# thelaycon/lazzaro

Measured on AMD Instinct MI355X. Metric: search_memories QPS + recall@10 on 10M x d=768 index; consolidate turns/sec, higher is better.
Workload: dtype bf16 encoder; int8 scan -> bf16 re-score -> fp32 re-rank; 1 GPU; global_batch=1024, seq_len=32, parallelism=tenant-dp1

## Files before the change

### csrc/kernels/search.hip

```cpp
#include "lzk_tile.h"

#include <cstdlib>

namespace {

constexpr int BM = 128;
constexpr int BN = 128;
constexpr int BK = 64;
constexpr int NT = 256;
constexpr int TILE_ELEMS = BM * BK;

__device__ __forceinline__ int swz_off(int row, int kc) {
  return row * BK + ((kc ^ ((row >> 1) & 7)) << 3);
}

template <int K>
struct TopK {
  float s[K];
  int i[K];
  __device__ __forceinline__ void init() {
#pragma unroll
    for (int j = 0; j < K; ++j) { s[j] = LZK_NEG_INF; i[j] = -1; }
  }
  __device__ __forceinline__ void push(float v, int r) {
    if (v > s[K - 1]) {
#pragma unroll
      for (int j = K - 1; j > 0; --j) {
        bool up = v > s[j - 1];
        bool here = v > s[j];
        float ns = up ? s[j - 1] : (here ? v : s[j]);
        int ni = up ? i[j - 1] : (here ? r : i[j]);
        s[j] = ns; i[j] = ni;
      }
      if (v > s[0]) { s[0] = v; i[0] = r; }
    }
  }
};

template <int K, bool HAS_BIAS, bool HAS_LABEL, bool GLDS>
__global__ __launch_bounds__(NT, 2) void flat_topk_kernel(
    const u16* __restrict__ X, long ldx, int nrows,
    const u16* __restrict__ Qm, long ldq, int nq,
    const float* __restrict__ bias, const int* __restrict__ row_label,
    const int* __restrict__ q_label, float alpha, int D,
    int rows_per_chunk, int n_chunks, int n_qblocks,
    float* __restrict__ out_s, int* __restrict__ out_i, const int* __restrict__ q_active) {
  extern __shared__ __attribute__((aligned(16))) u16 smem[];
  const int tid = threadIdx.x;
  const int lane = tid & 63;
  const int wave = tid >> 6;
  const int wrow = wave >> 1, wcol = wave & 1;
  const int h = lane >> 5, l32 = lane & 31;

  const int logical = xcd_remap(blockIdx.x, gridDim.x);
  const int chunk = logical / n_qblocks;
  const int qb = logical % n_qblocks;
  if (chunk >= n_chunks) return;
  const int q0 = qb * BN;
  if (q_active) {
    int any = 0;
    for (int t = tid; t < BN; t += NT) any |= (q0 + t < nq) && q_active[q0 + t];
    if (!__syncthreads_or(any)) return;
  }
  const int row_lo = chunk * rows_per_chunk;
  const int row_hi = min(nrows, row_lo + rows_per_chunk);
  const int ntiles = (row_hi > row_lo) ? (row_hi - row_lo + BM - 1) / BM : 0;
  const int KSTEPS = D / BK;
  const int T = ntiles * KSTEPS;

  int qlab[2] = {-1, -1};
  if (HAS_LABEL) {
#pragma unroll
    for (int cb = 0; cb < 2; ++cb) {
      int q = q0 + wcol * 64 + cb * 32 + l32;
      qlab[cb] = (q < nq) ? q_label[q] : -1;
    }
  }

  TopK<K> top[2];
  top[0].init(); top[1].init();

  const int srow = tid >> 3;
  const int skc = tid & 7;
  const u16* xsrc[4];
  const u16* qsrc[4];
  int soff[4];
#pragma unroll
  for (int i = 0; i < 4; ++i) {
    int r = srow + 32 * i;
    int q = min(q0 + r, nq - 1);
    qsrc[i] = Qm + (long)q * ldq + skc * 8;
    soff[i] = swz_off(r, skc);
  }
  auto set_xsrc = [&](int rt) {
#pragma unroll
    for (int i = 0; i < 4; ++i) {
      int r = row_lo + rt * BM + srow + 32 * i;
      r = min(r, nrows - 1);
      xsrc[i] = X + (long)r * ldx + skc * 8;
    }
  };

  const int wave_u = __builtin_amdgcn_readfirstlane(wave);
  const u16* gx[4];
  const u16* gq[4];
  int gpiece[4];
#pragma unroll
  for (int i = 0; i < 4; ++i) {
    const int c = wave_u * 4 + i;
    const int row = 8 * c + (lane >> 3);
    const int kc = (lane & 7) ^ ((row >> 1) & 7);
    gq[i] = Qm + (long)min(q0 + row, nq - 1) * ldq + kc * 8;
    gx[i] = X;
    gpiece[i] = c * 512;
  }
  auto set_gx = [&](int rt_) {
#pragma unroll
    for (int i = 0; i < 4; ++i) {
      const int row = 8 * (wave_u * 4 + i) + (lane >> 3);
      const int kc = (lane & 7) ^ ((row >> 1) & 7);
      gx[i] = X + (long)min(row_lo + rt_ * BM + row, nrows - 1) * ldx + kc * 8;
    }
  };
  float* ebias_g = reinterpret_cast<float*>(smem + 4 * TILE_ELEMS);
  int* elab_g = reinterpret_cast<int*>(ebias_g + 2 * BM);
  auto gissue = [&](int buf, int ks_, int rt_) {
    u16* xs = smem + buf * 2 * TILE_ELEMS;
    u16* qs = xs + TILE_ELEMS;
#pragma unroll
    for (int i = 0; i < 4; ++i) {
      __builtin_amdgcn_global_load_lds((lzk::gbl_void_t*)(gx[i] + ks_ * BK), (lzk::lds_void_t*)(xs + gpiece[i]), 16, 0, 0);
      __builtin_amdgcn_global_load_lds((lzk::gbl_void_t*)(gq[i] + ks_ * BK), (lzk::lds_void_t*)(qs + gpiece[i]), 16, 0, 0);
    }
    if ((HAS_BIAS || HAS_LABEL) && ks_ == 0 && wave_u == 0) {
#pragma unroll
      for (int h2 = 0; h2 < 2; ++h2) {
        const int r = min(row_lo + rt_ * BM + h2 * 64 + lane, nrows - 1);
        if (HAS_BIAS)
          __builtin_amdgcn_global_load_lds((lzk::gbl_void_t*)(bias + r), (lzk::lds_void_t*)(ebias_g + (rt_ & 1) * BM + h2 * 64), 4, 0, 0);
        if (HAS_LABEL)
          __builtin_amdgcn_global_load_lds((lzk::gbl_void_t*)(row_label + r), (lzk::lds_void_t*)(elab_g + (rt_ & 1) * BM + h2 * 64), 4, 0, 0);
      }
    }
  };

  u16x8 rx[4], rq[4];
  float rbias = 0.f;
  int rlab = 0;
  float* ebias = reinterpret_cast<float*>(smem + 4 * TILE_ELEMS);
  int* elab = reinterpret_cast<int*>(ebias + 2 * BM);
  auto gload = [&](int ks, int rt_) {
#pragma unroll
    for (int i = 0; i < 4; ++i) {
      rx[i] = *reinterpret_cast<const u16x8*>(xsrc[i] + ks * BK);
      rq[i] = *reinterpret_cast<const u16x8*>(qsrc[i] + ks * BK);
    }
    if ((HAS_BIAS || HAS_LABEL) && ks == 0 && tid < BM) {
      int r = min(row_lo + rt_ * BM + tid, nrows - 1);
      if (HAS_BIAS) rbias = bias[r];
      if (HAS_LABEL) rlab = row_label[r];
    }
  };
  auto swrite = [&](int buf, int ks, int rt_) {
    u16* xs = smem + buf * 2 * TILE_ELEMS;
    u16* qs = xs + TILE_ELEMS;
#pragma unroll
    for (int i = 0; i < 4; ++i) {
      *reinterpret_cast<u16x8*>(xs + soff[i]) = rx[i];
      *reinterpret_cast<u16x8*>(qs + soff[i]) = rq[i];
    }
    if ((HAS_BIAS || HAS_LABEL) && ks == 0 && tid < BM) {
      if (HAS_BIAS) ebias[(rt_ & 1) * BM + tid] = rbias;
      if (HAS_LABEL) elab[(rt_ & 1) * BM + tid] = rlab;
    }
  };

  f32x16 acc[2][2];

  if (T > 0) {
    if (GLDS) {
      set_gx(0);
      gissue(0, 0, 0);
      lzk::vm_drain();
    } else {
      set_xsrc(0);
      gload(0, 0);
      swrite(0, 0, 0);
    }
  }
  __syncthreads();

  int rt = 0, ks = 0;
  for (int t = 0; t < T; ++t) {
    const bool has_next = (t + 1 < T);
    const int nks = (ks + 1 == KSTEPS) ? 0 : ks + 1;
    const int nrt = (ks + 1 == KSTEPS) ? rt + 1 : rt;
    if (has_next) {
      if (GLDS) {
        if (nks == 0) set_gx(nrt);
        gissue((t + 1) & 1, nks, nrt);
      } else {
        if (nks == 0) set_xsrc(nrt);
        gload(nks, nrt);
      }
    }
    if (ks == 0) {
#pragma unroll
      for (int a = 0; a < 2; ++a)
#pragma unroll
        for (int b = 0; b < 2; ++b)
#pragma unroll
          for (int e = 0; e < 16; ++e) acc[a][b][e] = 0.f;
    }
    if (GLDS) __builtin_amdgcn_s_setprio(1);
    {
      const u16* xs = smem + (t & 1) * 2 * TILE_ELEMS;
      const u16* qs = xs + TILE_ELEMS;
#pragma unroll
      for (int s = 0; s < BK / 16; ++s) {
        bf16x8 af[2], bfr[2];
#pragma unroll
        for (int rb = 0; rb < 2; ++rb) {
          int r = wrow * 64 + rb * 32 + l32;
          af[rb] = *reinterpret_cast<const bf16x8*>(xs + swz_off(r, 2 * s + h));
        }
#pragma unroll
        for (int cb = 0; cb < 2; ++cb) {
          int r = wcol * 64 + cb * 32 + l32;
          bfr[cb] = *reinterpret_cast<const bf16x8*>(qs + swz_off(r, 2 * s + h));
        }
#pragma unroll
        for (int rb = 0; rb < 2; ++rb)
#pragma unroll
          for (int cb = 0; cb < 2; ++cb)
            acc[rb][cb] = __builtin_amdgcn_mfma_f32_32x32x16_bf16(af[rb], bfr[cb], acc[rb][cb], 0, 0, 0);
      }
    }
    if (GLDS) __builtin_amdgcn_s_setprio(0);
    if (ks == KSTEPS - 1) {
      const int lrow0 = wrow * 64 + 4 * h;
      const int tile0 = row_lo + rt * BM + lrow0;
      const float* eb = ebias + (rt & 1) * BM + lrow0;
      const int* el = elab + (rt & 1) * BM + lrow0;
      const bool full_tile = row_lo + (rt + 1) * BM <= row_hi;
      auto score = [&](int rb, int cb, int e) -> float {
        float x = alpha * acc[rb][cb][e];
        if (HAS_BIAS) x += eb[rb * 32 + 8 * (e >> 2) + (e & 3)];
        bool ok = true;
        if (!full_tile) ok = tile0 + rb * 32 + (e & 3) + 8 * (e >> 2) < row_hi;
        if (HAS_LABEL) ok = ok && (qlab[cb] < 0 || el[rb * 32 + 8 * (e >> 2) + (e & 3)] == qlab[cb]);
        return ok ? x : LZK_NEG_INF;
      };
#pragma unroll
      for (int rb = 0; rb < 2; ++rb) {
#pragma unroll
        for (int cb = 0; cb < 2; ++cb) {
          float m = LZK_NEG_INF;
#pragma unroll
          for (int e = 0; e < 16; ++e) m = fmaxf(m, score(rb, cb, e));
          if (m > top[cb].s[K - 1]) {
#pragma unroll
            for (int e = 0; e < 16; ++e)
              top[cb].push(score(rb, cb, e), tile0 + rb * 32 + (e & 3) + 8 * (e >> 2));
          }
        }
      }
    }
    if (GLDS) {
      lzk::vm_drain();
    } else if (has_next) {
      swrite((t + 1) & 1, nks, nrt);
    }
    __syncthreads();
    ks = nks; rt = nrt;
  }

  float* ms = reinterpret_cast<float*>(smem);
  int* mi = reinterpret_cast<int*>(smem) + BN * 4 * K;
#pragma unroll
  for (int cb = 0; cb < 2; ++cb) {
    int ql = wcol * 64 + cb * 32 + l32;
    int li = wrow * 2 + h;
#pragma unroll
    for (int j = 0; j < K; ++j) {
      ms[(ql * 4 + li) * K + j] = top[cb].s[j];
      mi[(ql * 4 + li) * K + j] = top[cb].i[j];
    }
  }
  __syncthreads();
  if (tid < BN) {
    const int ql = tid;
    const int q = q0 + ql;
    if (q < nq) {
      int p0 = 0, p1 = 0, p2 = 0, p3 = 0;
      const float* bs = ms + ql * 4 * K;
      const int* bi = mi + ql * 4 * K;
      long obase = ((long)q * n_chunks + chunk) * K;
      for (int j = 0; j < K; ++j) {
        float bsv = LZK_NEG_INF; int biv = -1; int w = -1;
        if (p0 < K) { float s = bs[0 * K + p0]; int i = bi[0 * K + p0]; if (w < 0 || better(s, i, bsv, biv)) { bsv = s; biv = i; w = 0; } }
        if (p1 < K) { float s = bs[1 * K + p1]; int i = bi[1 * K + p1]; if (w < 0 || better(s, i, bsv, biv)) { bsv = s; biv = i; w = 1; } }
        if (p2 < K) { float s = bs[2 * K + p2]; int i = bi[2 * K + p2]; if (w < 0 || better(s, i, bsv, biv)) { bsv = s; biv = i; w = 2; } }
        if (p3 < K) { float s = bs[3 * K + p3]; int i = bi[3 * K + p3]; if (w < 0 || better(s, i, bsv, biv)) { bsv = s; biv = i; w = 3; } }
        p0 += (w == 0); p1 += (w == 1); p2 += (w == 2); p3 += (w == 3);
        out_s[obase + j] = bsv;
        out_i[obase + j] = (bsv == LZK_NEG_INF) ? -1 : biv;
      }
    }
  }
}

template <int K>
__global__ __launch_bounds__(256) void topk_merge_kernel(
    const float* __restrict__ ps, const int* __restrict__ pi, int ncand, int nq,
    int kout, long idx_offset, float* __restrict__ os, long* __restrict__ oi, const int* __restrict__ q_active) {
  const int lane = threadIdx.x & 63;
  const int q = blockIdx.x * 4 + (threadIdx.x >> 6);
  if (q >= nq) return;
  if (q_active && !q_active[q]) return;
  TopK<K> top;
  top.init();
  const float* s = ps + (long)q * ncand;
  const int* ix = pi + (long)q * ncand;
  for (int c = lane; c < ncand; c += 64) {
    float v = s[c];
    int r = ix[c];
    if (r < 0) continue;
    if (better(v, r, top.s[K - 1], top.i[K - 1] < 0 ? 0x7fffffff : top.i[K - 1])) {
#pragma unroll
      for (int j = K - 1; j > 0; --j) {
        int ij1 = top.i[j - 1] < 0 ? 0x7fffffff : top.i[j - 1];
        int ij = top.i[j] < 0 ? 0x7fffffff : top.i[j];
        bool up = better(v, r, top.s[j - 1], ij1);
        bool here = better(v, r, top.s[j], ij);
        float ns = up ? top.s[j - 1] : (here ? v : top.s[j]);
        int ni = up ? top.i[j - 1] : (here ? r : top.i[j]);
        top.s[j] = ns; top.i[j] = ni;
      }
      int i0 = top.i[0] < 0 ? 0x7fffffff : top.i[0];
      if (better(v, r, top.s[0], i0)) { top.s[0] = v; top.i[0] = r; }
    }
  }
// ... 144 lines not shown
  if (D % BK != 0 || nq <= 0 || nrows <= 0) return (int)hipErrorInvalidValue;
  hipStream_t st = (hipStream_t)stream;
  const u16* x = (const u16*)X;
  const u16* q = (const u16*)Qm;
#define LZK_KS(KK) return launch_flat<KK>(x, ldx, nrows, q, ldq, nq, bias, row_label, q_label, alpha, D, n_chunks, ps, pi, st, q_active)
  switch (kslot) {
    case 1: LZK_KS(1);
    case 2: LZK_KS(2);
    case 4: LZK_KS(4);
    case 8: LZK_KS(8);
    case 10: LZK_KS(10);
    case 16: LZK_KS(16);
    default: return (int)hipErrorInvalidValue;
  }
#undef LZK_KS
}

LZK_EXPORT int lzk_flat_topk_partial(const void* X, long ldx, int nrows, const void* Qm, long ldq,
                                     int nq, const float* bias, const int* row_label,
                                     const int* q_label, float alpha, int D, int kslot,
                                     int n_chunks, float* ps, int* pi, void* stream) {
  return flat_partial(X, ldx, nrows, Qm, ldq, nq, bias, row_label, q_label, alpha, D, kslot, n_chunks, ps, pi,
                      stream, nullptr);
}

LZK_EXPORT int lzk_flat_topk_partial_masked(const void* X, long ldx, int nrows, const void* Qm, long ldq, int nq,
                                            const float* bias, const int* row_label, const int* q_label,
                                            float alpha, int D, int kslot, int n_chunks, float* ps, int* pi,
                                            const int* q_active, void* stream) {
  return flat_partial(X, ldx, nrows, Qm, ldq, nq, bias, row_label, q_label, alpha, D, kslot, n_chunks, ps, pi,
                      stream, q_active);
}

static int topk_merge(const float* ps, const int* pi, int ncand, int nq, int kslot, int kout, long idx_offset,
                      float* os, long* oi, void* stream, const int* q_active) {
  hipStream_t st = (hipStream_t)stream;
  dim3 grid((nq + 3) / 4), block(256);
  if (kout > kslot) return (int)hipErrorInvalidValue;
#define LZK_M(KK) hipLaunchKernelGGL(topk_merge_kernel<KK>, grid, block, 0, st, ps, pi, ncand, nq, kout, idx_offset, os, oi, q_active)
  switch (kslot) {
    case 1: LZK_M(1); break;
    case 2: LZK_M(2); break;
    case 4: LZK_M(4); break;
    case 8: LZK_M(8); break;
    case 10: LZK_M(10); break;
    case 16: LZK_M(16); break;
    default: return (int)hipErrorInvalidValue;
  }
#undef LZK_M
  return (int)hipGetLastError();
}

LZK_EXPORT int lzk_topk_merge(const float* ps, const int* pi, int ncand, int nq, int kslot,
                              int kout, long idx_offset, float* os, long* oi, void* stream) {
  return topk_merge(ps, pi, ncand, nq, kslot, kout, idx_offset, os, oi, stream, nullptr);
}

LZK_EXPORT int lzk_topk_merge64(const float* ps, const long* pi, int ncand, int nq, int kout, float* os, long* oi,
                                void* stream) {
  if (nq <= 0) return 0;
  if (kout < 1 || ncand < 0) return (int)hipErrorInvalidValue;
  hipStream_t st = (hipStream_t)stream;
  dim3 grid((nq + 3) / 4), block(256);
#define LZK_M64(KK) hipLaunchKernelGGL(topk_merge64_kernel<KK>, grid, block, 0, st, ps, pi, ncand, nq, kout, os, oi)
  if (kout <= 4) LZK_M64(4);
  else if (kout <= 10) LZK_M64(10);
// ... 12 lines not shown
```

### csrc/kernels/search256.hip

```cpp
#include "lzk_g256.h"

#include <cstdlib>
#include <cfloat>
#include <map>
#include <mutex>

LZK_DEBUG_STATE(search256)

namespace {

using namespace g256;

constexpr int kStampTiles = 32;
__device__ unsigned long long* g_stamps = nullptr;

template <bool HAS_BIAS, bool HAS_LABEL>
__global__ __launch_bounds__(NT, 1) void flat_cand_kernel(
    const u16* __restrict__ X, long ldx, int nrows, const u16* __restrict__ Qm, long ldq, int nq, int D,
    const float* __restrict__ bias, const int* __restrict__ row_label, const int* __restrict__ q_label,
    float alpha, const float* __restrict__ thr, int n_qt, int cap, int* __restrict__ cnt,
    float* __restrict__ cs, int* __restrict__ ci) {
  extern __shared__ __attribute__((aligned(16))) u16 smem[];
  const int logical = xcd_remap(blockIdx.x, gridDim.x);
  const int rt = logical / n_qt, qt = logical % n_qt;
  const int r0 = rt * BM, q0 = qt * BN;

  Stager st;
  st.setup(X, ldx, r0, nrows, Qm, ldq, q0, nq);
  f32x4 acc[8][4];
  mainloop(smem, st, D / BK, acc);

  const int lane = threadIdx.x & 63;
  const int wave = __builtin_amdgcn_readfirstlane(threadIdx.x >> 6);
// ... 31 lines not shown
        s[e] = ok ? s[e] : LZK_NEG_INF;
        m = fmaxf(m, s[e]);
      }
      if (m >= th[j]) {
#pragma unroll
        for (int e = 0; e < 4; ++e) {
          if (s[e] >= th[j] && s[e] != LZK_NEG_INF) {
            const int pos = atomicAdd(cnt + qq[j], 1);
            if (pos < cap) {
              cs[(long)qq[j] * cap + pos] = s[e];
              ci[(long)qq[j] * cap + pos] = rb + e;
            }
          }
        }
      }
    }
  }
}

constexpr int EPI_OFF = 8 * HALF;
constexpr int EPI_ARRAYS = 7;
constexpr int CNT_OFF = EPI_OFF + 2 * EPI_ARRAYS * 256 * 2;
constexpr int CAND_P_LDS = LDS_BYTES + 2 * EPI_ARRAYS * 256 * 4 + 16;
typedef __attribute__((address_space(3))) int lds_int;

struct BlkCands {
  int4* buf;
  int cap;
  int* cnt;
  const float* rs = nullptr;
  const float* qs = nullptr;
};

__device__ __forceinline__ float i8_prod(int v, float rs) { return __fmul_rn((float)v, rs); }
__device__ __forceinline__ float i8_score(float al, float p, float b) { return __fmaf_rn(al, p, b); }

template <bool HAS_BIAS, bool HAS_LABEL, bool DUAL, int OPT = 0, class MMA = MmaBf16>
__global__ __launch_bounds__(NT, 1) void flat_cand_persistent_kernel(
    const u16* __restrict__ X, long ldx, int nrows, const u16* __restrict__ Qm, long ldq, int nq, int D,
    const float* __restrict__ bias, const int* __restrict__ row_label, const int* __restrict__ q_label,
    float alpha, const float* __restrict__ thr, int n_qt, int n_tiles, int cap, int* __restrict__ cnt,
    float* __restrict__ cs, int* __restrict__ ci, const float* __restrict__ thr2, int* __restrict__ cnt2,
    float* __restrict__ cs2, int* __restrict__ ci2, BlkCands blk) {
  static_assert(!DUAL || HAS_LABEL, "dual search needs labels");
  extern __shared__ __attribute__((aligned(16))) u16 smem[];
  float* epi = reinterpret_cast<float*>(smem + EPI_OFF);
  lds_int* lcnt = (lds_int*)(smem + CNT_OFF);
  if (threadIdx.x == 0) *lcnt = 0;
  const int lane = threadIdx.x & 63;
  const int wave = __builtin_amdgcn_readfirstlane(threadIdx.x >> 6);
  const int wr = wave >> 2, wc = wave & 3;
  const int KS = D / BK;

  TileWalk walk;
  walk.init(n_tiles);
  int tile = walk.next;
  if (!walk.valid(tile)) {
    if (threadIdx.x == 0) blk.cnt[blockIdx.x] = 0;
    return;
  }

  auto stage_epi = [&](int tl, int par) {
    const int r0 = (tl / n_qt) * BM, q0 = (tl % n_qt) * BN;
#pragma unroll
    for (int g = wave; g < 4 * EPI_ARRAYS; g += 8) {
      const int a = g >> 2, c = g & 3;
      const bool need = a == 0 || (a == 1 && HAS_BIAS) || ((a == 2 || a == 3) && HAS_LABEL) || (a == 4 && DUAL) ||
                        ((a == 5 || a == 6) && MMA::kInt);
// ... 1323 lines not shown
```

### lazzaro_amd/ops/search.py

```python
from __future__ import annotations

import os

import numpy as np
import torch

from . import _lib

TARGET_WGS = 512


def _ref_topk(X, Q, k, bias=None, row_label=None, q_label=None, alpha=1.0, idx_offset=0,
              chunk=1 << 16):
    nq = Q.shape[0]
    n = X.shape[0]
    dev = X.device
    best_s = torch.full((nq, 0), float("-inf"), device=dev)
    best_i = torch.zeros((nq, 0), dtype=torch.long, device=dev)
    Qf = Q.float()
    for c0 in range(0, n, chunk):
        c1 = min(n, c0 + chunk)
        s = alpha * (Qf @ X[c0:c1].float().T)
        if bias is not None:
            s = s + bias[c0:c1].float()[None, :]
# ... 102 lines not shown
        return s[:, 0], i[:, 0].to(torch.int32)
    assert X.dtype == torch.bfloat16 and Q.dtype == torch.bfloat16
    assert X.shape[1] == D and D % 64 == 0 and X.stride(1) == 1 and Q.stride(1) == 1
    dev = X.device
    if N == 0 or nq == 0:
        return torch.full((nq,), float("-inf"), device=dev), torch.full((nq,), -1, dtype=torch.int32, device=dev)
    ws = torch.empty(nq, dtype=torch.int64, device=dev)
    score = torch.empty(nq, dtype=torch.float32, device=dev)
    row = torch.empty(nq, dtype=torch.int32, device=dev)
    _lib.check(_lib.lib().lzk_flat_top1(X.data_ptr(), X.stride(0), N, Q.data_ptr(), Q.stride(0), nq, D, ws.data_ptr(),
                                        score.data_ptr(), row.data_ptr(), _lib.stream_ptr(dev)), "lzk_flat_top1")
    return score, row


def _flat_topk_lane(X, Q, k, kslot, bias, row_label, q_label, alpha, idx_offset, n_chunks):
    L = _lib.lib()
    nq, D = Q.shape
    N = X.shape[0]
    if n_chunks:
        rpc = -(-(-(-N // n_chunks)) // 128) * 128
        nch = -(-N // rpc)
    else:
        nch = L.lzk_flat_topk_chunks(N, nq, TARGET_WGS)
    dev = X.device
    part = nq * nch * kslot
    ws = _ws.get(dev, part * 8)
    ps = ws[: part * 4].view(torch.float32)
    pi = ws[part * 4: part * 8].view(torch.int32)
    st = _lib.stream_ptr(dev)
    rc = L.lzk_flat_topk_partial(X.data_ptr(), X.stride(0), N, Q.data_ptr(), Q.stride(0), nq,
                                 _lib.ptr(bias), _lib.ptr(row_label), _lib.ptr(q_label),
                                 float(alpha), D, kslot, nch, ps.data_ptr(), pi.data_ptr(), st)
    _lib.check(rc, "lzk_flat_topk_partial")
    ncand = nch * kslot
    G = _merge_groups(nq, nch)
    if G > 1:
        os1 = torch.empty((nq * G, kslot), dtype=torch.float32, device=dev)
        oi1 = torch.empty((nq * G, kslot), dtype=torch.long, device=dev)
        _lib.check(L.lzk_topk_merge(ps.data_ptr(), pi.data_ptr(), ncand // G, nq * G, kslot, kslot, 0,
                                    os1.data_ptr(), oi1.data_ptr(), st), "lzk_topk_merge")
        ps, pi, ncand = os1, oi1.to(torch.int32), G * kslot
    os_ = torch.empty((nq, k), dtype=torch.float32, device=dev)
    oi = torch.empty((nq, k), dtype=torch.long, device=dev)
    rc = L.lzk_topk_merge(ps.data_ptr(), pi.data_ptr(), ncand, nq, kslot, int(k),
                          int(idx_offset), os_.data_ptr(), oi.data_ptr(), st)
    _lib.check(rc, "lzk_topk_merge")
    return os_, oi


def _merge_groups(nq: int, nch: int) -> int:
    if nq >= 64 or nch < 16:
        return 1
    for G in range(min(64, nch // 8, 512 // max(nq, 1)), 1, -1):
        if nch % G == 0:
            return G
    return 1


def _sample_threshold(X, Q, k, kslot, bias, row_label, q_label, alpha, S):
    N = X.shape[0]
    bs = bias[:N:S].contiguous() if bias is not None else None
    ls = row_label[:N:S].contiguous() if row_label is not None else None
    ts, _ = _flat_topk_lane(X[::S], Q, kslot, kslot, bs, ls, q_label, alpha, 0, None)
    thr = ts[:, k - 1].contiguous()
    thr = thr - 2e-4 * (1.0 + thr.abs())
    return torch.nan_to_num(thr, nan=float("-inf"))
# ... 232 lines not shown


def quantize_i8_rows(x: torch.Tensor, out: torch.Tensor = None, scale_out: torch.Tensor = None):
    xf = x.float()
    amax = xf.abs().amax(1)
    s = torch.where(amax > 0, amax / 127.0, torch.zeros_like(amax))
    den = torch.where(amax > 0, s, torch.ones_like(amax))
    q = torch.round(xf / den[:, None]).clamp_(-127, 127).to(torch.int8)
    if out is not None:
        out[:, : q.shape[1]] = q
        q = out
    if scale_out is not None:
        scale_out.copy_(s)
        s = scale_out
    return q, s


def i8_query(q16: torch.Tensor, d: int, sumsq: torch.Tensor, n_sumsq: int, smax: torch.Tensor, alpha: float,
             z: float, xn: float = 1.0):
    nq, Dp = q16.shape
    dev = q16.device
    q8 = torch.empty((nq, Dp), dtype=torch.int8, device=dev)
    qs = torch.empty(nq, dtype=torch.float32, device=dev)
    margin = torch.empty(nq, dtype=torch.float32, device=dev)
    margin_rig = torch.empty(nq, dtype=torch.float32, device=dev)
    q16 = q16.contiguous()
    _lib.check(_lib.lib().lzk_i8_query(q16.data_ptr(), q16.stride(0), nq, Dp, int(d), sumsq.data_ptr(),
                                       1.0 / max(int(n_sumsq), 1), smax.data_ptr(), abs(float(alpha)), float(z),
                                       float(xn), q8.data_ptr(), q8.stride(0), qs.data_ptr(), margin.data_ptr(),
                                       margin_rig.data_ptr(), _lib.stream_ptr(dev)), "lzk_i8_query")
    return q8, qs, margin, margin_rig


def flat_topk_i8(X8: torch.Tensor, rscale: torch.Tensor, Q8: torch.Tensor, qscale: torch.Tensor,
                 X16: torch.Tensor, Q16: torch.Tensor, k: int, *, bias=None, alpha: float = 1.0, margin=None,
                 margin_rig=None):
    L = _lib.lib()
    nq, Dp = Q16.shape
    N = X16.shape[0]
    kslot = L.lzk_flat_topk_kslot(int(k))
    assert kslot > 0 and X8.dtype == torch.int8 and Q8.dtype == torch.int8 and Dp % 128 == 0 and Dp <= 1024
    assert X8.shape[1] == Dp and X8.stride(1) == 1 and Q8.stride(1) == 1 and X8.shape[0] >= N
    assert rscale.dtype == torch.float32 and qscale.dtype == torch.float32 and rscale.shape[0] >= N
    assert alpha > 0
    dev = X16.device
    if margin_rig is None:
        margin_rig = margin
    narrow = nq < NARROW_MAX_Q and SCAN8_NARROW and Dp % 64 == 0
    S = max(1, min(CAND_STRIDE_NARROW if narrow else CAND_STRIDE, N // max(16 * kslot, 1)))
    J = SPEC_J_NARROW if narrow else SPEC_J
    spec = 0 < J < k and S >= SPEC_MIN_STRIDE
    bs = bias[:N:S].contiguous() if bias is not None else None
    ts, _ = _flat_topk_lane(X16[::S], Q16, kslot, kslot, bs, None, None, alpha, 0, None)
    cap = max(NARROW_CAP if narrow else 2048, 16 * kslot * S)
    cnt, cs, ci = _cand_lists(dev, nq, cap, 0, zero=False)
    thr = torch.empty(nq, dtype=torch.float32, device=dev)
    cert = torch.empty(nq, dtype=torch.float32, device=dev)
    mg = margin.float().contiguous() if margin is not None else None
    mr = margin_rig.float().contiguous() if margin_rig is not None else None
    _lib.check(L.lzk_thr_prep(ts.data_ptr(), ts.stride(0), (J if spec else k) - 1, _lib.ptr(mg), _lib.ptr(mr), nq,
                              thr.data_ptr(), cert.data_ptr(), cnt.data_ptr(), _lib.stream_ptr(dev)), "lzk_thr_prep")
    qs = qscale.contiguous()
    need = torch.empty(nq, dtype=torch.int32, device=dev)
    chk = (cert, k, cap + 1, need)
    if narrow:
        _scan8_narrow(X8[:N], rscale[:N], Q8, qs, bias, alpha, thr, kslot, 2 * S, cap, (cnt, cs, ci))
    else:
        grid = L.lzk_cand_grid_f8(N, nq)
        bbuf, bcap, bcnt = _blk_records(dev, grid, nq, kslot, 2 * S, 1)
        st = _lib.stream_ptr(dev)
        _lib.check(L.lzk_flat_cand_i8(X8.data_ptr(), X8.stride(0), N, Q8.data_ptr(), Q8.stride(0), nq, Dp,
                                      _lib.ptr(bias), rscale.data_ptr(), qs.data_ptr(), float(alpha), thr.data_ptr(),
                                      cap, cnt.data_ptr(), cs.data_ptr(), ci.data_ptr(), bbuf.data_ptr(), bcap,
                                      bcnt.data_ptr(), st), "lzk_flat_cand_i8")
        _lib.check(L.lzk_cand_gather(bbuf.data_ptr(), bcap, bcnt.data_ptr(), grid, cap, nq, cnt.data_ptr(),
                                     cs.data_ptr(), ci.data_ptr(), None, None, None, st), "lzk_cand_gather")
    _rescore_above_cut(X16, Q16, k, kslot, bias, alpha, margin_rig, cnt, cs, ci, cap, chk=chk)
    return _select_with_fallback(X16, Q16, k, kslot, bias, None, None, alpha, 0, cnt, cs, ci, cap, need=need)


def _cert_tau(thr: torch.Tensor, margin_rig: torch.Tensor, floor: float = None,
              floor_tol: float = 0.0) -> torch.Tensor:
    t = thr + margin_rig if margin_rig is not None else thr
    fl_ok = (t <= float(floor) + float(floor_tol)) if floor is not None else None
    t = t + 1e-6 * (1.0 + t.abs())
    if fl_ok is not None:
# ... 367 lines not shown
```

Baseline: 85750 queries/s.

## Compute strided sample top-k threshold with int8 MFMA directly on X8

Adds a sample_topk_i8 kernel that scores every S-th row of the int8 index with i32 MFMA and per-row/per-query scales, then merges the partials. This replaces the bf16 sampled top-k, which first materialised a strided copy of the bias and read the bf16 rows X16[::S]. The intent is to halve the bytes read by the threshold-estimation pass and drop the strided gather and copy. In exchange the thresholds now come from quantized scores, which may differ slightly from the bf16 ones and can change how many candidates pass the filter. It is enabled by default through an environment flag.

```diff
diff --git a/csrc/include/lzk_i8score.h b/csrc/include/lzk_i8score.h
--- /dev/null
+++ b/csrc/include/lzk_i8score.h
@@ -0,0 +1,5 @@
+#pragma once
+#include "lzk_common.h"
+
+__device__ __forceinline__ float i8_prod(int v, float rs) { return __fmul_rn((float)v, rs); }
+__device__ __forceinline__ float i8_score(float al, float p, float b) { return __fmaf_rn(al, p, b); }
diff --git a/csrc/kernels/search.hip b/csrc/kernels/search.hip
--- a/csrc/kernels/search.hip
+++ b/csrc/kernels/search.hip
@@ -1,4 +1,5 @@
 #include "lzk_tile.h"
+#include "lzk_i8score.h"
 
 #include <cstdlib>
 
@@ -37,244 +38,13 @@
   }
 };
 
-template <int K, bool HAS_BIAS, bool HAS_LABEL, bool GLDS>
-__global__ __launch_bounds__(NT, 2) void flat_topk_kernel(
-    const u16* __restrict__ X, long ldx, int nrows,
-    const u16* __restrict__ Qm, long ldq, int nq,
-    const float* __restrict__ bias, const int* __restrict__ row_label,
-    const int* __restrict__ q_label, float alpha, int D,
-    int rows_per_chunk, int n_chunks, int n_qblocks,
-    float* __restrict__ out_s, int* __restrict__ out_i, const int* __restrict__ q_active) {
-  extern __shared__ __attribute__((aligned(16))) u16 smem[];
+template <int K>
+__device__ __forceinline__ void merge_lane_lists(u16* smem, const TopK<K> (&top)[2], int q0, int nq, int n_chunks,
+                                                 int chunk, float* __restrict__ out_s, int* __restrict__ out_i) {
   const int tid = threadIdx.x;
-  const int lane = tid & 63;
-  const int wave = tid >> 6;
+  const int lane = tid & 63, wave = tid >> 6;
   const int wrow = wave >> 1, wcol = wave & 1;
   const int h = lane >> 5, l32 = lane & 31;
-
-  const int logical = xcd_remap(blockIdx.x, gridDim.x);
-  const int chunk = logical / n_qblocks;
-  const int qb = logical % n_qblocks;
-  if (chunk >= n_chunks) return;
-  const int q0 = qb * BN;
-  if (q_active) {
-    int any = 0;
-    for (int t = tid; t < BN; t += NT) any |= (q0 + t < nq) && q_active[q0 + t];
-    if (!__syncthreads_or(any)) return;
-  }
-  const int row_lo = chunk * rows_per_chunk;
-  const int row_hi = min(nrows, row_lo + rows_per_chunk);
-  const int ntiles = (row_hi > row_lo) ? (row_hi - row_lo + BM - 1) / BM : 0;
-  const int KSTEPS = D / BK;
-  const int T = ntiles * KSTEPS;
-
-  int qlab[2] = {-1, -1};
-  if (HAS_LABEL) {
-#pragma unroll
-    for (int cb = 0; cb < 2; ++cb) {
-      int q = q0 + wcol * 64 + cb * 32 + l32;
-      qlab[cb] = (q < nq) ? q_label[q] : -1;
-    }
-  }
-
-  TopK<K> top[2];
-  top[0].init(); top[1].init();
-
-  const int srow = tid >> 3;
-  const int skc = tid & 7;
-  const u16* xsrc[4];
-  const u16* qsrc[4];
-  int soff[4];
-#pragma unroll
-  for (int i = 0; i < 4; ++i) {
-    int r = srow + 32 * i;
-    int q = min(q0 + r, nq - 1);
-    qsrc[i] = Qm + (long)q * ldq + skc * 8;
-    soff[i] = swz_off(r, skc);
-  }
-  auto set_xsrc = [&](int rt) {
-#pragma unroll
-    for (int i = 0; i < 4; ++i) {
-      int r = row_lo + rt * BM + srow + 32 * i;
-      r = min(r, nrows - 1);
-      xsrc[i] = X + (long)r * ldx + skc * 8;
-    }
-  };
-
-  const int wave_u = __builtin_amdgcn_readfirstlane(wave);
-  const u16* gx[4];
-  const u16* gq[4];
-  int gpiece[4];
-#pragma unroll
-  for (int i = 0; i < 4; ++i) {
-    const int c = wave_u * 4 + i;
-    const int row = 8 * c + (lane >> 3);
-    const int kc = (lane & 7) ^ ((row >> 1) & 7);
-    gq[i] = Qm + (long)min(q0 + row, nq - 1) * ldq + kc * 8;
-    gx[i] = X;
-    gpiece[i] = c * 512;
-  }
-  auto set_gx = [&](int rt_) {
-#pragma unroll
-    for (int i = 0; i < 4; ++i) {
-      const int row = 8 * (wave_u * 4 + i) + (lane >> 3);
-      const int kc = (lane & 7) ^ ((row >> 1) & 7);
-      gx[i] = X + (long)min(row_lo + rt_ * BM + row, nrows - 1) * ldx + kc * 8;
-    }
-  };
-  float* ebias_g = reinterpret_cast<float*>(smem + 4 * TILE_ELEMS);
-  int* elab_g = reinterpret_cast<int*>(ebias_g + 2 * BM);
-  auto gissue = [&](int buf, int ks_, int rt_) {
-    u16* xs = smem + buf * 2 * TILE_ELEMS;
-    u16* qs = xs + TILE_ELEMS;
-#pragma unroll
-    for (int i = 0; i < 4; ++i) {
-      __builtin_amdgcn_global_load_lds((lzk::gbl_void_t*)(gx[i] + ks_ * BK), (lzk::lds_void_t*)(xs + gpiece[i]), 16, 0, 0);
-      __builtin_amdgcn_global_load_lds((lzk::gbl_void_t*)(gq[i] + ks_ * BK), (lzk::lds_void_t*)(qs + gpiece[i]), 16, 0, 0);
-    }
-    if ((HAS_BIAS || HAS_LABEL) && ks_ == 0 && wave_u == 0) {
-#pragma unroll
-      for (int h2 = 0; h2 < 2; ++h2) {
-        const int r = min(row_lo + rt_ * BM + h2 * 64 + lane, nrows - 1);
-        if (HAS_BIAS)
-          __builtin_amdgcn_global_load_lds((lzk::gbl_void_t*)(bias + r), (lzk::lds_void_t*)(ebias_g + (rt_ & 1) * BM + h2 * 64), 4, 0, 0);
-        if (HAS_LABEL)
-          __builtin_amdgcn_global_load_lds((lzk::gbl_void_t*)(row_label + r), (lzk::lds_void_t*)(elab_g + (rt_ & 1) * BM + h2 * 64), 4, 0, 0);
-      }
-    }
-  };
-
-  u16x8 rx[4], rq[4];
-  float rbias = 0.f;
-  int rlab = 0;
-  float* ebias = reinterpret_cast<float*>(smem + 4 * TILE_ELEMS);
-  int* elab = reinterpret_cast<int*>(ebias + 2 * BM);
-  auto gload = [&](int ks, int rt_) {
-#pragma unroll
-    for (int i = 0; i < 4; ++i) {
-      rx[i] = *reinterpret_cast<const u16x8*>(xsrc[i] + ks * BK);
-      rq[i] = *reinterpret_cast<const u16x8*>(qsrc[i] + ks * BK);
-    }
-    if ((HAS_BIAS || HAS_LABEL) && ks == 0 && tid < BM) {
-      int r = min(row_lo + rt_ * BM + tid, nrows - 1);
-      if (HAS_BIAS) rbias = bias[r];
-      if (HAS_LABEL) rlab = row_label[r];
-    }
-  };
-  auto swrite = [&](int buf, int ks, int rt_) {
-    u16* xs = smem + buf * 2 * TILE_ELEMS;
-    u16* qs = xs + TILE_ELEMS;
-#pragma unroll
-    for (int i = 0; i < 4; ++i) {
-      *reinterpret_cast<u16x8*>(xs + soff[i]) = rx[i];
-      *reinterpret_cast<u16x8*>(qs + soff[i]) = rq[i];
-    }
-    if ((HAS_BIAS || HAS_LABEL) && ks == 0 && tid < BM) {
-      if (HAS_BIAS) ebias[(rt_ & 1) * BM + tid] = rbias;
-      if (HAS_LABEL) elab[(rt_ & 1) * BM + tid] = rlab;
-    }
-  };
-
-  f32x16 acc[2][2];
-
-  if (T > 0) {
-    if (GLDS) {
-      set_gx(0);
-      gissue(0, 0, 0);
-      lzk::vm_drain();
-    } else {
-      set_xsrc(0);
-      gload(0, 0);
-      swrite(0, 0, 0);
-    }
-  }
-  __syncthreads();
-
-  int rt = 0, ks = 0;
-  for (int t = 0; t < T; ++t) {
-    const bool has_next = (t + 1 < T);
-    const int nks = (ks + 1 == KSTEPS) ? 0 : ks + 1;
-    const int nrt = (ks + 1 == KSTEPS) ? rt + 1 : rt;
-    if (has_next) {
-      if (GLDS) {
-        if (nks == 0) set_gx(nrt);
-        gissue((t + 1) & 1, nks, nrt);
-      } else {
-        if (nks == 0) set_xsrc(nrt);
-        gload(nks, nrt);
-      }
-    }
-    if (ks == 0) {
-#pragma unroll
-      for (int a = 0; a < 2; ++a)
-#pragma unroll
-        for (int b = 0; b < 2; ++b)
-#pragma unroll
-          for (int e = 0; e < 16; ++e) acc[a][b][e] = 0.f;
-    }
-    if (GLDS) __builtin_amdgcn_s_setprio(1);
-    {
-      const u16* xs = smem + (t & 1) * 2 * TILE_ELEMS;
-      const u16* qs = xs + TILE_ELEMS;
-#pragma unroll
-      for (int s = 0; s < BK / 16; ++s) {
-        bf16x8 af[2], bfr[2];
-#pragma unroll
-        for (int rb = 0; rb < 2; ++rb) {
-          int r = wrow * 64 + rb * 32 + l32;
-          af[rb] = *reinterpret_cast<const bf16x8*>(xs + swz_off(r, 2 * s + h));
-        }
-#pragma unroll
-        for (int cb = 0; cb < 2; ++cb) {
-          int r = wcol * 64 + cb * 32 + l32;
-          bfr[cb] = *reinterpret_cast<const bf16x8*>(qs + swz_off(r, 2 * s + h));
-        }
-#pragma unroll
-        for (int rb = 0; rb < 2; ++rb)
-#pragma unroll
-          for (int cb = 0; cb < 2; ++cb)
-            acc[rb][cb] = __builtin_amdgcn_mfma_f32_32x32x16_bf16(af[rb], bfr[cb], acc[rb][cb], 0, 0, 0);
-      }
-    }
-    if (GLDS) __builtin_amdgcn_s_setprio(0);
-    if (ks == KSTEPS - 1) {
-      const int lrow0 = wrow * 64 + 4 * h;
-      const int tile0 = row_lo + rt * BM + lrow0;
-      const float* eb = ebias + (rt & 1) * BM + lrow0;
-      const int* el = elab + (rt & 1) * BM + lrow0;
-      const bool full_tile = row_lo + (rt + 1) * BM <= row_hi;
-      auto score = [&](int rb, int cb, int e) -> float {
-        float x = alpha * acc[rb][cb][e];
-        if (HAS_BIAS) x += eb[rb * 32 + 8 * (e >> 2) + (e & 3)];
-        bool ok = true;
-        if (!full_tile) ok = tile0 + rb * 32 + (e & 3) + 8 * (e >> 2) < row_hi;
-        if (HAS_LABEL) ok = ok && (qlab[cb] < 0 || el[rb * 32 + 8 * (e >> 2) + (e & 3)] == qlab[cb]);
-        return ok ? x : LZK_NEG_INF;
-      };
-#pragma unroll
-      for (int rb = 0; rb < 2; ++rb) {
-#pragma unroll
-        for (int cb = 0; cb < 2; ++cb) {
-          float m = LZK_NEG_INF;
-#pragma unroll
-          for (int e = 0; e < 16; ++e) m = fmaxf(m, score(rb, cb, e));
-          if (m > top[cb].s[K - 1]) {
-#pragma unroll
-            for (int e = 0; e < 16; ++e)
-              top[cb].push(score(rb, cb, e), tile0 + rb * 32 + (e & 3) + 8 * (e >> 2));
-          }
-        }
-      }
-    }
-    if (GLDS) {
-      lzk::vm_drain();
-    } else if (has_next) {
-      swrite((t + 1) & 1, nks, nrt);
-    }
-    __syncthreads();
-    ks = nks; rt = nrt;
-  }
-
   float* ms = reinterpret_cast<float*>(smem);
   int* mi = reinterpret_cast<int*>(smem) + BN * 4 * K;
 #pragma unroll
@@ -308,6 +78,409 @@
       }
     }
   }
+}
+
+template <int K, bool HAS_BIAS, bool HAS_LABEL, bool GLDS>
+__global__ __launch_bounds__(NT, 2) void flat_topk_kernel(
+    const u16* __restrict__ X, long ldx, int nrows,
+    const u16* __restrict__ Qm, long ldq, int nq,
+    const float* __restrict__ bias, const int* __restrict__ row_label,
+    const int* __restrict__ q_label, float alpha, int D,
+    int rows_per_chunk, int n_chunks, int n_qblocks,
+    float* __restrict__ out_s, int* __restrict__ out_i, const int* __restrict__ q_active) {
+  extern __shared__ __attribute__((aligned(16))) u16 smem[];
+  const int tid = threadIdx.x;
+  const int lane = tid & 63;
+  const int wave = tid >> 6;
+  const int wrow = wave >> 1, wcol = wave & 1;
+  const int h = lane >> 5, l32 = lane & 31;
+
+  const int logical = xcd_remap(blockIdx.x, gridDim.x);
+  const int chunk = logical / n_qblocks;
+  const int qb = logical % n_qblocks;
+  if (chunk >= n_chunks) return;
+  const int q0 = qb * BN;
+  if (q_active) {
+    int any = 0;
+    for (int t = tid; t < BN; t += NT) any |= (q0 + t < nq) && q_active[q0 + t];
+    if (!__syncthreads_or(any)) return;
+  }
+  const int row_lo = chunk * rows_per_chunk;
+  const int row_hi = min(nrows, row_lo + rows_per_chunk);
+  const int ntiles = (row_hi > row_lo) ? (row_hi - row_lo + BM - 1) / BM : 0;
+  const int KSTEPS = D / BK;
+  const int T = ntiles * KSTEPS;
+
+  int qlab[2] = {-1, -1};
+  if (HAS_LABEL) {
+#pragma unroll
+    for (int cb = 0; cb < 2; ++cb) {
+      int q = q0 + wcol * 64 + cb * 32 + l32;
+      qlab[cb] = (q < nq) ? q_label[q] : -1;
+    }
+  }
+
+  TopK<K> top[2];
+  top[0].init(); top[1].init();
+
+  const int srow = tid >> 3;
+  const int skc = tid & 7;
+  const u16* xsrc[4];
+  const u16* qsrc[4];
+  int soff[4];
+#pragma unroll
+  for (int i = 0; i < 4; ++i) {
+    int r = srow + 32 * i;
+    int q = min(q0 + r, nq - 1);
+    qsrc[i] = Qm + (long)q * ldq + skc * 8;
+    soff[i] = swz_off(r, skc);
+  }
+  auto set_xsrc = [&](int rt) {
+#pragma unroll
+    for (int i = 0; i < 4; ++i) {
+      int r = row_lo + rt * BM + srow + 32 * i;
+      r = min(r, nrows - 1);
+      xsrc[i] = X + (long)r * ldx + skc * 8;
+    }
+  };
+
+  const int wave_u = __builtin_amdgcn_readfirstlane(wave);
+  const u16* gx[4];
+  const u16* gq[4];
+  int gpiece[4];
+#pragma unroll
+  for (int i = 0; i < 4; ++i) {
+    const int c = wave_u * 4 + i;
+    const int row = 8 * c + (lane >> 3);
+    const int kc = (lane & 7) ^ ((row >> 1) & 7);
+    gq[i] = Qm + (long)min(q0 + row, nq - 1) * ldq + kc * 8;
+    gx[i] = X;
+    gpiece[i] = c * 512;
+  }
+  auto set_gx = [&](int rt_) {
+#pragma unroll
+    for (int i = 0; i < 4; ++i) {
+      const int row = 8 * (wave_u * 4 + i) + (lane >> 3);
+      const int kc = (lane & 7) ^ ((row >> 1) & 7);
+      gx[i] = X + (long)min(row_lo + rt_ * BM + row, nrows - 1) * ldx + kc * 8;
+    }
+  };
+  float* ebias_g = reinterpret_cast<float*>(smem + 4 * TILE_ELEMS);
+  int* elab_g = reinterpret_cast<int*>(ebias_g + 2 * BM);
+  auto gissue = [&](int buf, int ks_, int rt_) {
+    u16* xs = smem + buf * 2 * TILE_ELEMS;
+    u16* qs = xs + TILE_ELEMS;
+#pragma unroll
+    for (int i = 0; i < 4; ++i) {
+      __builtin_amdgcn_global_load_lds((lzk::gbl_void_t*)(gx[i] + ks_ * BK), (lzk::lds_void_t*)(xs + gpiece[i]), 16, 0, 0);
+      __builtin_amdgcn_global_load_lds((lzk::gbl_void_t*)(gq[i] + ks_ * BK), (lzk::lds_void_t*)(qs + gpiece[i]), 16, 0, 0);
+    }
+    if ((HAS_BIAS || HAS_LABEL) && ks_ == 0 && wave_u == 0) {
+#pragma unroll
+      for (int h2 = 0; h2 < 2; ++h2) {
+        const int r = min(row_lo + rt_ * BM + h2 * 64 + lane, nrows - 1);
+        if (HAS_BIAS)
+          __builtin_amdgcn_global_load_lds((lzk::gbl_void_t*)(bias + r), (lzk::lds_void_t*)(ebias_g + (rt_ & 1) * BM + h2 * 64), 4, 0, 0);
+        if (HAS_LABEL)
+          __builtin_amdgcn_global_load_lds((lzk::gbl_void_t*)(row_label + r), (lzk::lds_void_t*)(elab_g + (rt_ & 1) * BM + h2 * 64), 4, 0, 0);
+      }
+    }
+  };
+
+  u16x8 rx[4], rq[4];
+  float rbias = 0.f;
+  int rlab = 0;
+  float* ebias = reinterpret_cast<float*>(smem + 4 * TILE_ELEMS);
+  int* elab = reinterpret_cast<int*>(ebias + 2 * BM);
+  auto gload = [&](int ks, int rt_) {
+#pragma unroll
+    for (int i = 0; i < 4; ++i) {
+      rx[i] = *reinterpret_cast<const u16x8*>(xsrc[i] + ks * BK);
+      rq[i] = *reinterpret_cast<const u16x8*>(qsrc[i] + ks * BK);
+    }
+    if ((HAS_BIAS || HAS_LABEL) && ks == 0 && tid < BM) {
+      int r = min(row_lo + rt_ * BM + tid, nrows - 1);
+      if (HAS_BIAS) rbias = bias[r];
+      if (HAS_LABEL) rlab = row_label[r];
+    }
+  };
+  auto swrite = [&](int buf, int ks, int rt_) {
+    u16* xs = smem + buf * 2 * TILE_ELEMS;
+    u16* qs = xs + TILE_ELEMS;
+#pragma unroll
+    for (int i = 0; i < 4; ++i) {
+      *reinterpret_cast<u16x8*>(xs + soff[i]) = rx[i];
+      *reinterpret_cast<u16x8*>(qs + soff[i]) = rq[i];
+    }
+    if ((HAS_BIAS || HAS_LABEL) && ks == 0 && tid < BM) {
+      if (HAS_BIAS) ebias[(rt_ & 1) * BM + tid] = rbias;
+      if (HAS_LABEL) elab[(rt_ & 1) * BM + tid] = rlab;
+    }
+  };
+
+  f32x16 acc[2][2];
+
+  if (T > 0) {
+    if (GLDS) {
+      set_gx(0);
+      gissue(0, 0, 0);
+      lzk::vm_drain();
+    } else {
+      set_xsrc(0);
+      gload(0, 0);
+      swrite(0, 0, 0);
+    }
+  }
+  __syncthreads();
+
+  int rt = 0, ks = 0;
+  for (int t = 0; t < T; ++t) {
+    const bool has_next = (t + 1 < T);
+    const int nks = (ks + 1 == KSTEPS) ? 0 : ks + 1;
+    const int nrt = (ks + 1 == KSTEPS) ? rt + 1 : rt;
+    if (has_next) {
+      if (GLDS) {
+        if (nks == 0) set_gx(nrt);
+        gissue((t + 1) & 1, nks, nrt);
+      } else {
+        if (nks == 0) set_xsrc(nrt);
+        gload(nks, nrt);
+      }
+    }
+    if (ks == 0) {
+#pragma unroll
+      for (int a = 0; a < 2; ++a)
+#pragma unroll
+        for (int b = 0; b < 2; ++b)
+#pragma unroll
+          for (int e = 0; e < 16; ++e) acc[a][b][e] = 0.f;
+    }
+    if (GLDS) __builtin_amdgcn_s_setprio(1);
+    {
+      const u16* xs = smem + (t & 1) * 2 * TILE_ELEMS;
+      const u16* qs = xs + TILE_ELEMS;
+#pragma unroll
+      for (int s = 0; s < BK / 16; ++s) {
+        bf16x8 af[2], bfr[2];
+#pragma unroll
+        for (int rb = 0; rb < 2; ++rb) {
+          int r = wrow * 64 + rb * 32 + l32;
+          af[rb] = *reinterpret_cast<const bf16x8*>(xs + swz_off(r, 2 * s + h));
+        }
+#pragma unroll
+        for (int cb = 0; cb < 2; ++cb) {
+          int r = wcol * 64 + cb * 32 + l32;
+          bfr[cb] = *reinterpret_cast<const bf16x8*>(qs + swz_off(r, 2 * s + h));
+        }
+#pragma unroll
+        for (int rb = 0; rb < 2; ++rb)
+#pragma unroll
+          for (int cb = 0; cb < 2; ++cb)
+            acc[rb][cb] = __builtin_amdgcn_mfma_f32_32x32x16_bf16(af[rb], bfr[cb], acc[rb][cb], 0, 0, 0);
+      }
+    }
+    if (GLDS) __builtin_amdgcn_s_setprio(0);
+    if (ks == KSTEPS - 1) {
+      const int lrow0 = wrow * 64 + 4 * h;
+      const int tile0 = row_lo + rt * BM + lrow0;
+      const float* eb = ebias + (rt & 1) * BM + lrow0;
+      const int* el = elab + (rt & 1) * BM + lrow0;
+      const bool full_tile = row_lo + (rt + 1) * BM <= row_hi;
+      auto score = [&](int rb, int cb, int e) -> float {
+        float x = alpha * acc[rb][cb][e];
+        if (HAS_BIAS) x += eb[rb * 32 + 8 * (e >> 2) + (e & 3)];
+        bool ok = true;
+        if (!full_tile) ok = tile0 + rb * 32 + (e & 3) + 8 * (e >> 2) < row_hi;
+        if (HAS_LABEL) ok = ok && (qlab[cb] < 0 || el[rb * 32 + 8 * (e >> 2) + (e & 3)] == qlab[cb]);
+        return ok ? x : LZK_NEG_INF;
+      };
+#pragma unroll
+      for (int rb = 0; rb < 2; ++rb) {
+#pragma unroll
+        for (int cb = 0; cb < 2; ++cb) {
+          float m = LZK_NEG_INF;
+#pragma unroll
+          for (int e = 0; e < 16; ++e) m = fmaxf(m, score(rb, cb, e));
+          if (m > top[cb].s[K - 1]) {
+#pragma unroll
+            for (int e = 0; e < 16; ++e)
+              top[cb].push(score(rb, cb, e), tile0 + rb * 32 + (e & 3) + 8 * (e >> 2));
+          }
+        }
+      }
+    }
+    if (GLDS) {
+      lzk::vm_drain();
+    } else if (has_next) {
+      swrite((t + 1) & 1, nks, nrt);
+    }
+    __syncthreads();
+    ks = nks; rt = nrt;
+  }
+
+  merge_lane_lists<K>(smem, top, q0, nq, n_chunks, chunk, out_s, out_i);
+}
+
+template <int K, bool HAS_BIAS>
+__global__ __launch_bounds__(NT, 2) void sample_topk_i8_kernel(
+    const int8_t* __restrict__ X, long ldx, int ns, int S,
+    const int8_t* __restrict__ Qm, long ldq, int nq,
+    const float* __restrict__ rscale, const float* __restrict__ qscale, const float* __restrict__ bias,
+    float alpha, int D, int rows_per_chunk, int n_chunks, int n_qblocks,
+    float* __restrict__ out_s, int* __restrict__ out_i) {
+  typedef int i32x4 __attribute__((ext_vector_type(4)));
+  typedef int i32x16 __attribute__((ext_vector_type(16)));
+  constexpr int BKB = 2 * BK;
+  extern __shared__ __attribute__((aligned(16))) u16 smem[];
+  const int tid = threadIdx.x;
+  const int lane = tid & 63;
+  const int wave = tid >> 6;
+  const int wrow = wave >> 1, wcol = wave & 1;
+  const int h = lane >> 5, l32 = lane & 31;
+
+  const int logical = xcd_remap(blockIdx.x, gridDim.x);
+  const int chunk = logical / n_qblocks;
+  const int qb = logical % n_qblocks;
+  if (chunk >= n_chunks) return;
+  const int q0 = qb * BN;
+  const int row_lo = chunk * rows_per_chunk;
+  const int row_hi = min(ns, row_lo + rows_per_chunk);
+  const int ntiles = (row_hi > row_lo) ? (row_hi - row_lo + BM - 1) / BM : 0;
+  const int KSTEPS = D / BKB;
+  const int T = ntiles * KSTEPS;
+
+  float al[2];
+#pragma unroll
+  for (int cb = 0; cb < 2; ++cb) al[cb] = alpha * qscale[min(q0 + wcol * 64 + cb * 32 + l32, nq - 1)];
+
+  TopK<K> top[2];
+  top[0].init(); top[1].init();
+
+  const int wave_u = __builtin_amdgcn_readfirstlane(wave);
+  const int8_t* gx[4];
+  const int8_t* gq[4];
+  int gpiece[4];
+#pragma unroll
+  for (int i = 0; i < 4; ++i) {
+    const int c = wave_u * 4 + i;
+    const int row = 8 * c + (lane >> 3);
+    const int kc = (lane & 7) ^ ((row >> 1) & 7);
+    gq[i] = Qm + (long)min(q0 + row, nq - 1) * ldq + kc * 16;
+    gx[i] = X;
+    gpiece[i] = c * 512;
+  }
+  auto set_gx = [&](int rt_) {
+#pragma unroll
+    for (int i = 0; i < 4; ++i) {
+      const int row = 8 * (wave_u * 4 + i) + (lane >> 3);
+      const int kc = (lane & 7) ^ ((row >> 1) & 7);
+      gx[i] = X + (long)min(row_lo + rt_ * BM + row, ns - 1) * S * ldx + kc * 16;
+    }
+  };
+  float* ebias = reinterpret_cast<float*>(smem + 4 * TILE_ELEMS);
+  float* ers = ebias + 2 * BM;
+  auto gissue = [&](int buf, int ks_, int rt_) {
+    u16* xs = smem + buf * 2 * TILE_ELEMS;
+    u16* qs = xs + TILE_ELEMS;
+#pragma unroll
+    for (int i = 0; i < 4; ++i) {
+      __builtin_amdgcn_global_load_lds((lzk::gbl_void_t*)(gx[i] + ks_ * BKB), (lzk::lds_void_t*)(xs + gpiece[i]), 16, 0, 0);
+      __builtin_amdgcn_global_load_lds((lzk::gbl_void_t*)(gq[i] + ks_ * BKB), (lzk::lds_void_t*)(qs + gpiece[i]), 16, 0, 0);
+    }
+    if (ks_ == 0 && wave_u == 0) {
+#pragma unroll
+      for (int h2 = 0; h2 < 2; ++h2) {
+        const long r = (long)min(row_lo + rt_ * BM + h2 * 64 + lane, ns - 1) * S;
+        __builtin_amdgcn_global_load_lds((lzk::gbl_void_t*)(rscale + r), (lzk::lds_void_t*)(ers + (rt_ & 1) * BM + h2 * 64), 4, 0, 0);
+        if (HAS_BIAS)
+          __builtin_amdgcn_global_load_lds((lzk::gbl_void_t*)(bias + r), (lzk::lds_void_t*)(ebias + (rt_ & 1) * BM + h2 * 64), 4, 0, 0);
+      }
+    }
+  };
+
+  i32x16 acc[2][2];
+
+  if (T > 0) {
+    set_gx(0);
+    gissue(0, 0, 0);
+    lzk::vm_drain();
+  }
+  __syncthreads();
+
+  int rt = 0, ks = 0;
+  for (int t = 0; t < T; ++t) {
+    const bool has_next = (t + 1 < T);
+    const int nks = (ks + 1 == KSTEPS) ? 0 : ks + 1;
+    const int nrt = (ks + 1 == KSTEPS) ? rt + 1 : rt;
+    if (has_next) {
+      if (nks == 0) set_gx(nrt);
+      gissue((t + 1) & 1, nks, nrt);
+    }
+    if (ks == 0) {
+#pragma unroll
+      for (int a = 0; a < 2; ++a)
+#pragma unroll
+        for (int b = 0; b < 2; ++b)
+#pragma unroll
+          for (int e = 0; e < 16; ++e) acc[a][b][e] = 0;
+    }
+    __builtin_amdgcn_s_setprio(1);
+    {
+      const u16* xs = smem + (t & 1) * 2 * TILE_ELEMS;
+      const u16* qs = xs + TILE_ELEMS;
+#pragma unroll
+      for (int s = 0; s < BKB / 32; ++s) {
+        i32x4 af[2], bfr[2];
+#pragma unroll
+        for (int rb = 0; rb < 2; ++rb) {
+          int r = wrow * 64 + rb * 32 + l32;
+          af[rb] = *reinterpret_cast<const i32x4*>(xs + swz_off(r, 2 * s + h));
+        }
+#pragma unroll
+        for (int cb = 0; cb < 2; ++cb) {
+          int r = wcol * 64 + cb * 32 + l32;
+          bfr[cb] = *reinterpret_cast<const i32x4*>(qs + swz_off(r, 2 * s + h));
+        }
+#pragma unroll
+        for (int rb = 0; rb < 2; ++rb)
+#pragma unroll
+          for (int cb = 0; cb < 2; ++cb)
+            acc[rb][cb] = __builtin_amdgcn_mfma_i32_32x32x32_i8(af[rb], bfr[cb], acc[rb][cb], 0, 0, 0);
+      }
+    }
+    __builtin_amdgcn_s_setprio(0);
+    if (ks == KSTEPS - 1) {
+      const int lrow0 = wrow * 64 + 4 * h;
+      const int tile0 = row_lo + rt * BM + lrow0;
+      const float* eb = ebias + (rt & 1) * BM + lrow0;
+      const float* er = ers + (rt & 1) * BM + lrow0;
+      const bool full_tile = row_lo + (rt + 1) * BM <= row_hi;
+      auto score = [&](int rb, int cb, int e) -> float {
+        const int lr = rb * 32 + 8 * (e >> 2) + (e & 3);
+        const float x = i8_score(al[cb], i8_prod(acc[rb][cb][e], er[lr]), HAS_BIAS ? eb[lr] : 0.f);
+        const bool ok = full_tile || tile0 + lr < row_hi;
+        return ok ? x : LZK_NEG_INF;
+      };
+#pragma unroll
+      for (int rb = 0; rb < 2; ++rb) {
+#pragma unroll
+        for (int cb = 0; cb < 2; ++cb) {
+          float m = LZK_NEG_INF;
+#pragma unroll
+          for (int e = 0; e < 16; ++e) m = fmaxf(m, score(rb, cb, e));
+          if (m > top[cb].s[K - 1]) {
+#pragma unroll
+            for (int e = 0; e < 16; ++e)
+              top[cb].push(score(rb, cb, e), (tile0 + rb * 32 + (e & 3) + 8 * (e >> 2)) * S);
+          }
+        }
+      }
+    }
+    lzk::vm_drain();
+    __syncthreads();
+    ks = nks; rt = nrt;
+  }
+  merge_lane_lists<K>(smem, top, q0, nq, n_chunks, chunk, out_s, out_i);
 }
 
 template <int K>
@@ -518,6 +691,41 @@
                       stream, q_active);
 }
 
+LZK_EXPORT int lzk_sample_topk_i8(const void* X8, long ldx, int nrows, int S, const void* Q8, long ldq, int nq,
+                                  const float* rscale, const float* qscale, const float* bias, float alpha, int D,
+                                  int kslot, int n_chunks, float* ps, int* pi, void* stream) {
+  if (D % (2 * BK) != 0 || D > 1024 || nq <= 0 || nrows <= 0 || S <= 0 || n_chunks <= 0) return (int)hipErrorInvalidValue;
+  if (ldx % 16 != 0 || ldq % 16 != 0 || ldx < D || ldq < D || ((uintptr_t)X8 | (uintptr_t)Q8) % 16 != 0)
+    return (int)hipErrorInvalidValue;
+  if (!rscale || !qscale) return (int)hipErrorInvalidValue;
+  hipStream_t st = (hipStream_t)stream;
+  const int ns = (int)(((long)nrows + S - 1) / S);
+  const int n_qblocks = (nq + BN - 1) / BN;
+  const int rows_per_chunk = ((ns + n_chunks - 1) / n_chunks + BM - 1) / BM * BM;
+  n_chunks = (ns + rows_per_chunk - 1) / rows_per_chunk;
+  dim3 grid(n_qblocks * n_chunks);
+#define LZK_SGO(KK, B) do { \
+  size_t lds = (size_t)2 * 2 * TILE_ELEMS * sizeof(u16) + 2 * BM * 8; \
+  if ((size_t)BN * 4 * KK * 8 > lds) lds = (size_t)BN * 4 * KK * 8; \
+  (void)hipFuncSetAttribute((const void*)sample_topk_i8_kernel<KK, B>, hipFuncAttributeMaxDynamicSharedMemorySize, (int)lds); \
+  hipLaunchKernelGGL((sample_topk_i8_kernel<KK, B>), grid, dim3(NT), lds, st, (const int8_t*)X8, ldx, ns, S, \
+                     (const int8_t*)Q8, ldq, nq, rscale, qscale, bias, alpha, D, rows_per_chunk, n_chunks, n_qblocks, \
+                     ps, pi); } while (0)
+#define LZK_SKS(KK) if (bias) LZK_SGO(KK, true); else LZK_SGO(KK, false); break
+  switch (kslot) {
+    case 1: LZK_SKS(1);
+    case 2: LZK_SKS(2);
+    case 4: LZK_SKS(4);
+    case 8: LZK_SKS(8);
+    case 10: LZK_SKS(10);
+    case 16: LZK_SKS(16);
+    default: return (int)hipErrorInvalidValue;
+  }
+#undef LZK_SKS
+#undef LZK_SGO
+  return (int)hipGetLastError();
+}
+
 static int topk_merge(const float* ps, const int* pi, int ncand, int nq, int kslot, int kout, long idx_offset,
                       float* os, long* oi, void* stream, const int* q_active) {
   hipStream_t st = (hipStream_t)stream;
diff --git a/csrc/kernels/search256.hip b/csrc/kernels/search256.hip
--- a/csrc/kernels/search256.hip
+++ b/csrc/kernels/search256.hip
@@ -1,4 +1,5 @@
 #include "lzk_g256.h"
+#include "lzk_i8score.h"
 
 #include <cstdlib>
 #include <cfloat>
@@ -96,8 +97,6 @@
   const float* qs = nullptr;
 };
 
-__device__ __forceinline__ float i8_prod(int v, float rs) { return __fmul_rn((float)v, rs); }
-__device__ __forceinline__ float i8_score(float al, float p, float b) { return __fmaf_rn(al, p, b); }
 
 template <bool HAS_BIAS, bool HAS_LABEL, bool DUAL, int OPT = 0, class MMA = MmaBf16>
 __global__ __launch_bounds__(NT, 1) void flat_cand_persistent_kernel(
diff --git a/lazzaro_amd/ops/search.py b/lazzaro_amd/ops/search.py
--- a/lazzaro_amd/ops/search.py
+++ b/lazzaro_amd/ops/search.py
@@ -158,6 +158,13 @@
                                  _lib.ptr(bias), _lib.ptr(row_label), _lib.ptr(q_label),
                                  float(alpha), D, kslot, nch, ps.data_ptr(), pi.data_ptr(), st)
     _lib.check(rc, "lzk_flat_topk_partial")
+    return _merge_partials(ps, pi, nch, nq, kslot, k, idx_offset)
+
+
+def _merge_partials(ps, pi, nch, nq, kslot, k, idx_offset):
+    L = _lib.lib()
+    dev = ps.device
+    st = _lib.stream_ptr(dev)
     ncand = nch * kslot
     G = _merge_groups(nq, nch)
     if G > 1:
@@ -456,6 +463,39 @@
     return q8, qs, margin, margin_rig
 
 
+I8_SAMPLE = os.environ.get("LZK_I8_SAMPLE", "1") != "0"
+_lib.register("lzk_sample_topk_i8", _lib.I, [_lib.P, _lib.L, _lib.I, _lib.I, _lib.P, _lib.L, _lib.I, _lib.P, _lib.P,
+                                             _lib.P, _lib.F, _lib.I, _lib.I, _lib.I, _lib.P, _lib.P, _lib.P])
+
+
+def sample_topk_i8(X8: torch.Tensor, rscale: torch.Tensor, Q8: torch.Tensor, qscale: torch.Tensor, kslot: int,
+                   S: int, *, bias=None, alpha: float = 1.0, n_chunks: int = None):
+    L = _lib.lib()
+    nq, Dp = Q8.shape
+    N = X8.shape[0]
+    dev = X8.device
+    assert X8.dtype == torch.int8 and Q8.dtype == torch.int8 and Dp % 128 == 0 and Dp <= 1024 and X8.shape[1] == Dp
+    assert X8.stride(1) == 1 and Q8.stride(1) == 1 and N > 0 and nq > 0 and S >= 1
+    assert rscale.dtype == torch.float32 and rscale.stride(0) == 1 and rscale.shape[0] >= N
+    assert bias is None or (bias.dtype == torch.float32 and bias.stride(0) == 1 and bias.shape[0] >= N)
+    qs = qscale.contiguous()
+    assert qs.dtype == torch.float32 and qs.shape[0] == nq
+    ns = -(-N // S)
+    if n_chunks:
+        rpc = -(-(-(-ns // n_chunks)) // 128) * 128
+        nch = -(-ns // rpc)
+    else:
+        nch = L.lzk_flat_topk_chunks(ns, nq, TARGET_WGS)
+    part = nq * nch * kslot
+    ws = _ws.get(dev, part * 8)
+    ps = ws[: part * 4].view(torch.float32)
+    pi = ws[part * 4: part * 8].view(torch.int32)
+    _lib.check(L.lzk_sample_topk_i8(X8.data_ptr(), X8.stride(0), N, int(S), Q8.data_ptr(), Q8.stride(0), nq,
+                                    rscale.data_ptr(), qs.data_ptr(), _lib.ptr(bias), float(alpha), Dp, kslot, nch,
+                                    ps.data_ptr(), pi.data_ptr(), _lib.stream_ptr(dev)), "lzk_sample_topk_i8")
+    return _merge_partials(ps, pi, nch, nq, kslot, kslot, 0)
+
+
 def flat_topk_i8(X8: torch.Tensor, rscale: torch.Tensor, Q8: torch.Tensor, qscale: torch.Tensor,
                  X16: torch.Tensor, Q16: torch.Tensor, k: int, *, bias=None, alpha: float = 1.0, margin=None,
                  margin_rig=None):
@@ -474,8 +514,11 @@
     S = max(1, min(CAND_STRIDE_NARROW if narrow else CAND_STRIDE, N // max(16 * kslot, 1)))
     J = SPEC_J_NARROW if narrow else SPEC_J
     spec = 0 < J < k and S >= SPEC_MIN_STRIDE
-    bs = bias[:N:S].contiguous() if bias is not None else None
-    ts, _ = _flat_topk_lane(X16[::S], Q16, kslot, kslot, bs, None, None, alpha, 0, None)
+    if I8_SAMPLE:
+        ts, _ = sample_topk_i8(X8[:N], rscale, Q8, qscale, kslot, S, bias=bias, alpha=alpha)
+    else:
+        bs = bias[:N:S].contiguous() if bias is not None else None
+        ts, _ = _flat_topk_lane(X16[::S], Q16, kslot, kslot, bs, None, None, alpha, 0, None)
     cap = max(NARROW_CAP if narrow else 2048, 16 * kslot * S)
     cnt, cs, ci = _cand_lists(dev, nq, cap, 0, zero=False)
     thr = torch.empty(nq, dtype=torch.float32, device=dev)
```

After: 86630 queries/s (median of 6 runs). 1.0% higher.
